# dalek-cryptography/bulletproofs

Measured on AMD Instinct MI355X. Metric: 64-bit rangeproof verifications/sec (batched), higher is better.
Workload: dtype u32 limbs (10x25.5-bit GF(2^255-19), 8x32-bit scalars mod l), u64 accumulators

## Files before the change

### bulletproofs_amd/csrc/k_rp34.hip

```cpp
#include <hip/hip_runtime.h>
#include "kernels.h"

using namespace bp;

#ifndef BP_STAGE3_WAVES
#define BP_STAGE3_WAVES 1
#endif
template <int FORM>
__global__ void __launch_bounds__(BP_BLOCK, FORM == 1 ? 1 : BP_STAGE3_WAVES) k_rp_stage3(uint32_t n_win, uint32_t nthreads_win, const vb_chunk *chunks, const ge_cached *tab,
                                                         const uint32_t *recoded, ge_ext *part, ge_cached *colc, uint32_t nthreads_exp,
                                                         rp_shape sh, fb_params prm, const uint32_t *fields, fb_digit *digits,
                                                         const uint32_t *status, uint32_t n_exp, uint32_t nthreads_rows, uint32_t lg_m, const ge_cached *tab_hi) {
    if (blockIdx.x < n_win) {
        const uint32_t tid = blockIdx.x * BP_BLOCK + threadIdx.x;
        if (tid < nthreads_win) vb_window_thread(tid, chunks, tab, recoded, part, colc, nullptr, tab_hi, sh.narrow_hi, (uint64_t)8 * sh.nproofs * sh.U);
    } else if (blockIdx.x < n_win + n_exp) {
        const uint32_t tid = (blockIdx.x - n_win) * BP_BLOCK + threadIdx.x;
        if (tid < nthreads_exp) {
            if (FORM == 1) rp_expand_b8_thread(tid, sh, prm, fields, digits, status);
            else if (FORM == 2) rp_expand_b1_thread(tid, sh, prm, fields, digits, status);
            else rp_expand_b4_thread(tid, sh, prm, fields, digits, status);
        }
    } else {
        const uint32_t tid = (blockIdx.x - n_win - n_exp) * BP_BLOCK + threadIdx.x;
        if (tid < nthreads_rows) rp_rows_thread(tid, sh, prm, lg_m, fields, digits, status);
    }
}
template __global__ void k_rp_stage3<0>(uint32_t, uint32_t, const vb_chunk *, const ge_cached *, const uint32_t *, ge_ext *, ge_cached *, uint32_t, rp_shape, fb_params,
                                        const uint32_t *, fb_digit *, const uint32_t *, uint32_t, uint32_t, uint32_t, const ge_cached *);
template __global__ void k_rp_stage3<1>(uint32_t, uint32_t, const vb_chunk *, const ge_cached *, const uint32_t *, ge_ext *, ge_cached *, uint32_t, rp_shape, fb_params,
                                        const uint32_t *, fb_digit *, const uint32_t *, uint32_t, uint32_t, uint32_t, const ge_cached *);
template __global__ void k_rp_stage3<2>(uint32_t, uint32_t, const vb_chunk *, const ge_cached *, const uint32_t *, ge_ext *, ge_cached *, uint32_t, rp_shape, fb_params,
                                        const uint32_t *, fb_digit *, const uint32_t *, uint32_t, uint32_t, uint32_t, const ge_cached *);

template <bool PAIRS>
__global__ void __attribute__((amdgpu_waves_per_eu(2, 2))) __launch_bounds__(BP_BLOCK) k_rp_exponents(uint32_t nthreads_exp, rp_shape sh, fb_params prm, const uint32_t *fields,
                                                                                                 fb_digit *digits, const uint32_t *status) {
    const uint32_t tid = blockIdx.x * BP_BLOCK + threadIdx.x;
    if (tid < nthreads_exp) {
        if (PAIRS) rp_expand_b8_thread(tid, sh, prm, fields, digits, status);
        else rp_expand_b4_thread(tid, sh, prm, fields, digits, status);
    }
}
template __global__ void k_rp_exponents<false>(uint32_t, rp_shape, fb_params, const uint32_t *, fb_digit *, const uint32_t *);
template __global__ void k_rp_exponents<true>(uint32_t, rp_shape, fb_params, const uint32_t *, fb_digit *, const uint32_t *);
__global__ void __attribute__((amdgpu_waves_per_eu(3, 3))) __launch_bounds__(BP_BLOCK) k_rp_exponents_w3(uint32_t nthreads_exp, rp_shape sh, fb_params prm, const uint32_t *fields,
                                                                                                    fb_digit *digits, const uint32_t *status) {
    const uint32_t tid = blockIdx.x * BP_BLOCK + threadIdx.x;
    if (tid < nthreads_exp) rp_expand_b8_thread(tid, sh, prm, fields, digits, status);
}

__global__ void __launch_bounds__(FB_BLOCK) k_rp_horner1(uint32_t nproofs, const ge_cached *colc, ge_ext *hq) {
    vb_horner_cached_thread(blockIdx.x * FB_BLOCK + threadIdx.x, nproofs, colc, hq);
}

template <bool R5>
__global__ void __launch_bounds__(FB_BLOCK) k_rp_horner_wide(uint32_t nproofs, const ge_cached *colc, const ge_cached *extra, uint32_t extra_stride, ge_ext *hq) {
    vb_horner_wide_thread<R5>(blockIdx.x * FB_BLOCK + threadIdx.x, nproofs, colc, extra, extra_stride, hq);
}
template __global__ void k_rp_horner_wide<false>(uint32_t, const ge_cached *, const ge_cached *, uint32_t, ge_ext *);
template __global__ void k_rp_horner_wide<true>(uint32_t, const ge_cached *, const ge_cached *, uint32_t, ge_ext *);

__device__ __forceinline__ void rp_fused_finish(uint32_t p, uint32_t nproofs, uint32_t nparts, const ge_ext *hq, const ge_ext *partial, uint32_t *fin_cnt, uint32_t *status,
                                                uint8_t *verdict, const rp_seg_tab &segs) {
    __threadfence();
    const uint32_t before = atomicAdd(fin_cnt + p, 1u);
    if (before != nparts) return;
    __threadfence();
    ge_ext acc = hq[p];
#pragma unroll 1
    for (uint32_t j = 0; j < nparts; j++) {
        const ge_ext q = partial[(uint64_t)j * nproofs + p];
        ge_add(acc, acc, q);
    }
    if (segs.n) {
        const rp_seg sg = rp_seg_lookup(segs, p);
        shared_finish_tail(p, p - sg.first, acc, status, nullptr, sg.verdict);
    } else {
        shared_finish_tail(p, acc, status, nullptr, verdict);
    }
    status[p] = 0;
    fin_cnt[p] = 0;
}
__device__ __forceinline__ void rp_walk_narrow(uint32_t L, fb_params prm, uint32_t nproofs, uint32_t nsplit, uint32_t npairs, const uint32_t *gen_ids,
                                               const fb_digit *digits, const fb_entry *table, ge_ext *partial, bool fused, const ge_ext *hq, uint32_t *fin_cnt,
                                               uint32_t *status, uint8_t *verdict, const rp_seg_tab &segs) {
    __shared__ ge_ext xch[FB_BLOCK];
    const uint32_t nsg = nsplit / FB_BLOCK, p = L / nsg, sg = L - p * nsg, lane = threadIdx.x, split = sg * FB_BLOCK + lane;
    const uint32_t per = (npairs + nsplit - 1) / nsplit;
    const uint32_t q0 = split * per, q1 = (q0 + per < npairs) ? q0 + per : npairs;
    ge_ext acc;
    fb_accum_point(acc, p, q0 < npairs ? q0 : npairs, q1, prm, nproofs, gen_ids, digits, table);
#pragma unroll 1
    for (uint32_t step = FB_BLOCK / 2; step >= 1; step >>= 1) {
        xch[lane] = acc;
        __syncthreads();
        if (lane < step) {
            const ge_ext q = xch[lane + step];
            ge_add(acc, acc, q);
        }
        __syncthreads();
    }
    if (lane == 0) {
        partial[(uint64_t)sg * nproofs + p] = acc;
        if (fused) rp_fused_finish(p, nproofs, nsg, hq, partial, fin_cnt, status, verdict, segs);
    }
}

template <int HL>
__global__ void __launch_bounds__(FB_BLOCK) k_rp_stage4(uint32_t n_hw, const uint32_t *chunk_first, const ge_ext *part, const ge_cached *colc,
                                                         ge_ext *hq, fb_params prm, uint32_t nproofs, uint32_t nblk_p, uint32_t nsplit,
                                                         uint32_t npairs, const uint32_t *gen_ids, const fb_digit *digits,
                                                         const fb_entry *table, ge_ext *partial, uint32_t walk_form, uint32_t *fin_cnt, uint32_t *status,
                                                         uint8_t *verdict, rp_seg_tab segs) {
    if (blockIdx.x < n_hw) {
            if (HL == 4) hq_horner_msm(blockIdx.x * 16 + (threadIdx.x >> 2), nproofs, colc, hq);
        else if (HL == 1) vb_horner_cached_thread(blockIdx.x * FB_BLOCK + threadIdx.x, nproofs, colc, hq);
        else {
            hw_colsum_horner_msm(blockIdx.x, chunk_first, part, hq + blockIdx.x, (walk_form & 8u) ? 4 : ((walk_form & 2u) ? 2 : 1));
            if (walk_form & 4u) {
                __threadfence();
                __syncthreads();
                if (threadIdx.x == 0) rp_fused_finish(blockIdx.x, nproofs, nsplit / FB_BLOCK, hq, partial, fin_cnt, status, verdict, segs);
            }
        }
        return;
    }
    if (HL == 64 && (walk_form & 1u)) {
        rp_walk_narrow(blockIdx.x - n_hw, prm, nproofs, nsplit, npairs, gen_ids, digits, table, partial, (walk_form & 4u) != 0, hq, fin_cnt, status, verdict, segs);
        return;
    }
    const uint32_t L = blockIdx.x - n_hw;
    uint32_t split, pblk;
    if ((nsplit & 7) == 0) {
        const uint32_t r = L & 7, rest = L >> 3;
        pblk = rest % nblk_p;
        split = r + 8 * (rest / nblk_p);
    } else {
        pblk = L % nblk_p;
        split = L / nblk_p;
    }
    const uint32_t p = pblk * FB_BLOCK + threadIdx.x;
    const uint32_t per = (npairs + nsplit - 1) / nsplit;
    const uint32_t q0 = split * per, q1 = (q0 + per < npairs) ? q0 + per : npairs;
    if (p < nproofs) fb_accum_thread(p, split, q0 < npairs ? q0 : npairs, q1, prm, nproofs, gen_ids, digits, table, partial);
}

template __global__ void k_rp_stage4<4>(uint32_t, const uint32_t *, const ge_ext *, const ge_cached *, ge_ext *, fb_params, uint32_t, uint32_t, uint32_t, uint32_t, const uint32_t *, const fb_digit *, const fb_entry *, ge_ext *, uint32_t, uint32_t *, uint32_t *, uint8_t *, rp_seg_tab);
template __global__ void k_rp_stage4<1>(uint32_t, const uint32_t *, const ge_ext *, const ge_cached *, ge_ext *, fb_params, uint32_t, uint32_t, uint32_t, uint32_t, const uint32_t *, const fb_digit *, const fb_entry *, ge_ext *, uint32_t, uint32_t *, uint32_t *, uint8_t *, rp_seg_tab);
template __global__ void k_rp_stage4<64>(uint32_t, const uint32_t *, const ge_ext *, const ge_cached *, ge_ext *, fb_params, uint32_t, uint32_t, uint32_t, uint32_t, const uint32_t *, const fb_digit *, const fb_entry *, ge_ext *, uint32_t, uint32_t *, uint32_t *, uint8_t *, rp_seg_tab);
```

### bulletproofs_amd/csrc/rangeproof.h

```cpp
#ifndef BPGPU_RANGEPROOF_H
#define BPGPU_RANGEPROOF_H
#include "keccak.h"
#include "rp_script.h"
#include "msm_fixed.h"
#include "sc25519.h"
#include "scinv.h"
#include "bucket.h"
#include "chacha20.h"

namespace bp {

#define BP_RP_MAX_K 16

#define BP_VERDICT_OK 0
#define BP_VERDICT_VERIFICATION 1
#define BP_VERDICT_FORMAT 2

struct rp_shape {
    uint32_t n, m, nm, k;
    uint32_t U;
    uint32_t proof_len;
    uint32_t nproofs;
    uint32_t shape_verdict;
    uint32_t radix5 = 0;
// ... 925 lines not shown
        else if (sh.n >= 32) { sum_2.v[0] = 0xffffffffu; sum_2.v[1] = (sh.n == 32) ? 0u : ((1u << (sh.n - 32)) - 1u); }
        else sum_2.v[0] = (1u << sh.n) - 1u;
        sc_sub(t1, z, zz);
        sc_to_mont28(dm, t1);
        sc28_montmul(dm, dm, sum_ym);
        sc_from_mont28(dl, dm);
        sc28 z3m, s2m;
        sc28_montmul(z3m, zzm, zm);
        sc_to_mont28(s2m, sum_2);
        sc28_montmul(z3m, z3m, s2m);
        sc28_montmul(z3m, z3m, sum_zm);
        sc_from_mont28(t1, z3m);
        sc_sub(dl, dl, t1);
        sc_sub(t1, dl, tx);
        sc_to_mont28(pm, t1);
        sc28_montmul(pm, cm, pm);
        sc_from_mont28(t1, pm);
        sc_add(t0, t0, t1);
        fb_recode(digits + ((uint64_t)1 * prm.nwin) * B + p, B, t0.v, prm);
    }
}

BP_HD void rp_two_pow_mont(sc28 &r, uint32_t i) {
    const sc28 T[64] = {
    {{0xcf5d3edu, 0x4305db8u, 0x676a4b2u, 0x80113d7u, 0x0622aafu, 0xfffeb21u, 0xfffffffu, 0xfffffffu, 0xfffffffu, 0x0000000u}},
    {{0xcf5d3edu, 0x73a89cbu, 0x550730cu, 0x0643d7fu, 0x0c44080u, 0xfffd642u, 0xfffffffu, 0xfffffffu, 0xfffffffu, 0x0000000u}},
    {{0xcf5d3edu, 0xd4ee1f1u, 0x3040fc0u, 0x12a90cfu, 0x1886c21u, 0xfffac84u, 0xfffffffu, 0xfffffffu, 0xfffffffu, 0x0000000u}},
    {{0xcf5d3edu, 0x977923du, 0xe6b4929u, 0x2b7376eu, 0x310c363u, 0xfff5908u, 0xfffffffu, 0xfffffffu, 0xfffffffu, 0x0000000u}},
    {{0xcf5d3edu, 0x1c8f2d5u, 0x539bbfbu, 0x5d084aeu, 0x62171e7u, 0xffeb210u, 0xfffffffu, 0xfffffffu, 0xfffffffu, 0x0000000u}},
    {{0xcf5d3edu, 0x26bb405u, 0x2d6a19eu, 0xc031f2du, 0xc42ceefu, 0xffd6420u, 0xfffffffu, 0xfffffffu, 0xfffffffu, 0x0000000u}},
    {{0xcf5d3edu, 0x3b13665u, 0xe106ce4u, 0x868542au, 0x8858900u, 0xffac841u, 0xfffffffu, 0xfffffffu, 0xfffffffu, 0x0000000u}},
    {{0xcf5d3edu, 0x63c3b25u, 0x4840370u, 0x132be26u, 0x10afd22u, 0xff59083u, 0xfffffffu, 0xfffffffu, 0xfffffffu, 0x0000000u}},
    {{0xcf5d3edu, 0xb5244a5u, 0x16b3088u, 0x2c7921du, 0x215e565u, 0xfeb2106u, 0xfffffffu, 0xfffffffu, 0xfffffffu, 0x0000000u}},
    {{0xcf5d3edu, 0x57e57a5u, 0xb398ab9u, 0x5f13a0au, 0x42bb5ebu, 0xfd6420cu, 0xfffffffu, 0xfffffffu, 0xfffffffu, 0x0000000u}},
    {{0xcf5d3edu, 0x9d67da5u, 0xed63f1au, 0xc4489e5u, 0x85756f7u, 0xfac8418u, 0xfffffffu, 0xfffffffu, 0xfffffffu, 0x0000000u}},
    {{0xcf5d3edu, 0x286c9a5u, 0x60fa7ddu, 0x8eb299cu, 0x0ae9910u, 0xf590831u, 0xfffffffu, 0xfffffffu, 0xfffffffu, 0x0000000u}},
    {{0xcf5d3edu, 0x3e761a5u, 0x4827962u, 0x2386909u, 0x15d1d42u, 0xeb21062u, 0xfffffffu, 0xfffffffu, 0xfffffffu, 0x0000000u}},
    {{0xcf5d3edu, 0x6a891a5u, 0x1681c6cu, 0x4d2e7e3u, 0x2ba25a5u, 0xd6420c4u, 0xfffffffu, 0xfffffffu, 0xfffffffu, 0x0000000u}},
    {{0xcf5d3edu, 0xc2af1a5u, 0xb336280u, 0xa07e596u, 0x574366bu, 0xac84188u, 0xfffffffu, 0xfffffffu, 0xfffffffu, 0x0000000u}},
    {{0xcf5d3edu, 0x72fb1a5u, 0xec9eea9u, 0x471e0fdu, 0xae857f8u, 0x5908310u, 0xfffffffu, 0xfffffffu, 0xfffffffu, 0x0000000u}},
    {{0xcf5d3edu, 0xd3931a5u, 0x5f706fau, 0x945d7ccu, 0x5d09b11u, 0xb210621u, 0xffffffeu, 0xfffffffu, 0xfffffffu, 0x0000000u}},
    {{0xcf5d3edu, 0x94c31a5u, 0x451379du, 0x2edc569u, 0xba12144u, 0x6420c42u, 0xffffffdu, 0xfffffffu, 0xfffffffu, 0x0000000u}},
    {{0xcf5d3edu, 0x17231a5u, 0x10598e3u, 0x63da0a3u, 0x7422da9u, 0xc841885u, 0xffffffau, 0xfffffffu, 0xfffffffu, 0x0000000u}},
    {{0xcf5d3edu, 0x1be31a5u, 0xa6e5b6eu, 0xcdd5716u, 0xe844673u, 0x908310au, 0xffffff5u, 0xfffffffu, 0xfffffffu, 0x0000000u}},
    {{0xcf5d3edu, 0x25631a5u, 0xd3fe084u, 0xa1cc3fdu, 0xd087808u, 0x2106215u, 0xfffffebu, 0xfffffffu, 0xfffffffu, 0x0000000u}},
    {{0xcf5d3edu, 0x38631a5u, 0x2e2eab0u, 0x49b9dccu, 0xa10db32u, 0x420c42bu, 0xfffffd6u, 0xfffffffu, 0xfffffffu, 0x0000000u}},
    {{0xcf5d3edu, 0x5e631a5u, 0xe28ff08u, 0x9995168u, 0x421a185u, 0x8418857u, 0xfffffacu, 0xfffffffu, 0xfffffffu, 0x0000000u}},
    {{0xcf5d3edu, 0xaa631a5u, 0x4b527b8u, 0x394b8a2u, 0x8432e2cu, 0x08310aeu, 0xfffff59u, 0xfffffffu, 0xfffffffu, 0x0000000u}},
    {{0xcf5d3edu, 0x42631a5u, 0x1cd7919u, 0x78b8715u, 0x0864779u, 0x106215du, 0xffffeb2u, 0xfffffffu, 0xfffffffu, 0x0000000u}},
    {{0xcf5d3edu, 0x72631a5u, 0xbfe1bdau, 0xf7923fau, 0x10c7a13u, 0x20c42bau, 0xffffd64u, 0xfffffffu, 0xfffffffu, 0x0000000u}},
    {{0xcf5d3edu, 0xd2631a5u, 0x05f615cu, 0xf545dc6u, 0x218df48u, 0x4188574u, 0xffffac8u, 0xfffffffu, 0xfffffffu, 0x0000000u}},
    {{0xcf5d3edu, 0x92631a5u, 0x921ec61u, 0xf0ad15cu, 0x431a9b2u, 0x8310ae8u, 0xffff590u, 0xfffffffu, 0xfffffffu, 0x0000000u}},
    {{0xcf5d3edu, 0x12631a5u, 0xaa7026bu, 0xe77b889u, 0x8633e86u, 0x06215d0u, 0xfffeb21u, 0xfffffffu, 0xfffffffu, 0x0000000u}},
    {{0xcf5d3edu, 0x12631a5u, 0xdb12e7eu, 0xd5186e3u, 0x0c6682eu, 0x0c42ba1u, 0xfffd642u, 0xfffffffu, 0xfffffffu, 0x0000000u}},
    {{0xcf5d3edu, 0x12631a5u, 0x3c586a4u, 0xb052398u, 0x18cbb7eu, 0x1885742u, 0xfffac84u, 0xfffffffu, 0xfffffffu, 0x0000000u}},
    {{0xcf5d3edu, 0x12631a5u, 0xfee36f0u, 0x66c5d00u, 0x319621eu, 0x310ae84u, 0xfff5908u, 0xfffffffu, 0xfffffffu, 0x0000000u}},
    {{0xcf5d3edu, 0x12631a5u, 0x83f9788u, 0xd3acfd2u, 0x632af5du, 0x6215d08u, 0xffeb210u, 0xfffffffu, 0xfffffffu, 0x0000000u}},
    {{0xcf5d3edu, 0x12631a5u, 0x8e258b8u, 0xad7b575u, 0xc6549dcu, 0xc42ba10u, 0xffd6420u, 0xfffffffu, 0xfffffffu, 0x0000000u}},
    {{0xcf5d3edu, 0x12631a5u, 0xa27db18u, 0x61180bbu, 0x8ca7edau, 0x8857421u, 0xffac841u, 0xfffffffu, 0xfffffffu, 0x0000000u}},
    {{0xcf5d3edu, 0x12631a5u, 0xcb2dfd8u, 0xc851747u, 0x194e8d5u, 0x10ae843u, 0xff59083u, 0xfffffffu, 0xfffffffu, 0x0000000u}},
    {{0xcf5d3edu, 0x12631a5u, 0x1c8e958u, 0x96c4460u, 0x329bcccu, 0x215d086u, 0xfeb2106u, 0xfffffffu, 0xfffffffu, 0x0000000u}},
    {{0xcf5d3edu, 0x12631a5u, 0xbf4fc58u, 0x33a9e90u, 0x65364bau, 0x42ba10cu, 0xfd6420cu, 0xfffffffu, 0xfffffffu, 0x0000000u}},
    {{0xcf5d3edu, 0x12631a5u, 0x04d2258u, 0x6d752f2u, 0xca6b495u, 0x8574218u, 0xfac8418u, 0xfffffffu, 0xfffffffu, 0x0000000u}},
    {{0xcf5d3edu, 0x12631a5u, 0x8fd6e58u, 0xe10bbb4u, 0x94d544bu, 0x0ae8431u, 0xf590831u, 0xfffffffu, 0xfffffffu, 0x0000000u}},
    {{0xcf5d3edu, 0x12631a5u, 0xa5e0658u, 0xc838d39u, 0x29a93b8u, 0x15d0863u, 0xeb21062u, 0xfffffffu, 0xfffffffu, 0x0000000u}},
    {{0xcf5d3edu, 0x12631a5u, 0xd1f3658u, 0x9693043u, 0x5351292u, 0x2ba10c6u, 0xd6420c4u, 0xfffffffu, 0xfffffffu, 0x0000000u}},
    {{0xcf5d3edu, 0x12631a5u, 0x2a19658u, 0x3347658u, 0xa6a1046u, 0x574218cu, 0xac84188u, 0xfffffffu, 0xfffffffu, 0x0000000u}},
    {{0xcf5d3edu, 0x12631a5u, 0xda65658u, 0x6cb0280u, 0x4d40badu, 0xae84319u, 0x5908310u, 0xfffffffu, 0xfffffffu, 0x0000000u}},
    {{0xcf5d3edu, 0x12631a5u, 0x3afd658u, 0xdf81ad2u, 0x9a8027bu, 0x5d08632u, 0xb210621u, 0xffffffeu, 0xfffffffu, 0x0000000u}},
    {{0xcf5d3edu, 0x12631a5u, 0xfc2d658u, 0xc524b74u, 0x34ff018u, 0xba10c65u, 0x6420c42u, 0xffffffdu, 0xfffffffu, 0x0000000u}},
    {{0xcf5d3edu, 0x12631a5u, 0x7e8d658u, 0x906acbau, 0x69fcb52u, 0x74218cau, 0xc841885u, 0xffffffau, 0xfffffffu, 0x0000000u}},
    {{0xcf5d3edu, 0x12631a5u, 0x834d658u, 0x26f6f45u, 0xd3f81c6u, 0xe843194u, 0x908310au, 0xffffff5u, 0xfffffffu, 0x0000000u}},
    {{0xcf5d3edu, 0x12631a5u, 0x8ccd658u, 0x540f45bu, 0xa7eeeadu, 0xd086329u, 0x2106215u, 0xfffffebu, 0xfffffffu, 0x0000000u}},
    {{0xcf5d3edu, 0x12631a5u, 0x9fcd658u, 0xae3fe87u, 0x4fdc87bu, 0xa10c653u, 0x420c42bu, 0xfffffd6u, 0xfffffffu, 0x0000000u}},
    {{0xcf5d3edu, 0x12631a5u, 0xc5cd658u, 0x62a12dfu, 0x9fb7c18u, 0x4218ca6u, 0x8418857u, 0xfffffacu, 0xfffffffu, 0x0000000u}},
    {{0xcf5d3edu, 0x12631a5u, 0x11cd658u, 0xcb63b90u, 0x3f6e351u, 0x843194du, 0x08310aeu, 0xfffff59u, 0xfffffffu, 0x0000000u}},
    {{0xcf5d3edu, 0x12631a5u, 0xa9cd658u, 0x9ce8cf0u, 0x7edb1c4u, 0x086329au, 0x106215du, 0xffffeb2u, 0xfffffffu, 0x0000000u}},
    {{0xcf5d3edu, 0x12631a5u, 0xd9cd658u, 0x3ff2fb1u, 0xfdb4eaau, 0x10c6534u, 0x20c42bau, 0xffffd64u, 0xfffffffu, 0x0000000u}},
    {{0xcf5d3edu, 0x12631a5u, 0x39cd658u, 0x8607534u, 0xfb68875u, 0x218ca69u, 0x4188574u, 0xffffac8u, 0xfffffffu, 0x0000000u}},
    {{0xcf5d3edu, 0x12631a5u, 0xf9cd658u, 0x1230038u, 0xf6cfc0cu, 0x43194d3u, 0x8310ae8u, 0xffff590u, 0xfffffffu, 0x0000000u}},
    {{0xcf5d3edu, 0x12631a5u, 0x79cd658u, 0x2a81642u, 0xed9e339u, 0x86329a7u, 0x06215d0u, 0xfffeb21u, 0xfffffffu, 0x0000000u}},
    {{0xcf5d3edu, 0x12631a5u, 0x79cd658u, 0x5b24255u, 0xdb3b193u, 0x0c6534fu, 0x0c42ba1u, 0xfffd642u, 0xfffffffu, 0x0000000u}},
    {{0xcf5d3edu, 0x12631a5u, 0x79cd658u, 0xbc69a7bu, 0xb674e47u, 0x18ca69fu, 0x1885742u, 0xfffac84u, 0xfffffffu, 0x0000000u}},
    {{0xcf5d3edu, 0x12631a5u, 0x79cd658u, 0x7ef4ac7u, 0x6ce87b0u, 0x3194d3fu, 0x310ae84u, 0xfff5908u, 0xfffffffu, 0x0000000u}},
    {{0xcf5d3edu, 0x12631a5u, 0x79cd658u, 0x040ab5fu, 0xd9cfa82u, 0x6329a7eu, 0x6215d08u, 0xffeb210u, 0xfffffffu, 0x0000000u}},
    {{0xcf5d3edu, 0x12631a5u, 0x79cd658u, 0x0e36c8fu, 0xb39e025u, 0xc6534fdu, 0xc42ba10u, 0xffd6420u, 0xfffffffu, 0x0000000u}},
    {{0xcf5d3edu, 0x12631a5u, 0x79cd658u, 0x228eeefu, 0x673ab6bu, 0x8ca69fbu, 0x8857421u, 0xffac841u, 0xfffffffu, 0x0000000u}},
    {{0xcf5d3edu, 0x12631a5u, 0x79cd658u, 0x4b3f3afu, 0xce741f7u, 0x194d3f6u, 0x10ae843u, 0xff59083u, 0xfffffffu, 0x0000000u}}};
    r = T[i & 63];
}
BP_HD void sc28_sub_lazy(sc28 &r, const sc28 &a, const sc28 &b) {
    const uint32_t L4[10] = {0x3d74fb4u, 0x498c697u, 0xe735960u, 0xe77a8bdu, 0x000537bu, 0u, 0u, 0u, 0u, 0x4u};
    int32_t cy = 0;
#pragma unroll
    for (int i = 0; i < 10; i++) {
        const int32_t t = (int32_t)a.v[i] - (int32_t)b.v[i] + (int32_t)L4[i] + cy;
        if (i < 9) {
            r.v[i] = (uint32_t)t & BP_M28;
            cy = t >> 28;
        } else {
            r.v[i] = (uint32_t)t;
        }
    }
}

BP_HD void rp_expand_b4_thread(uint32_t tid, rp_shape sh, fb_params prm, const uint32_t *fields, fb_digit *digits,
                               const uint32_t *status, sc *g_out = nullptr, sc *h_out = nullptr, uint32_t j_lo = 0, uint32_t j_hi = 4) {
    const uint32_t B = sh.nproofs, k = sh.k;
    const uint32_t t4 = tid / B, p = tid - t4 * B, i0 = 4 * t4;
    if (g_out) {
        for (int j = 0; j < 4; j++) {
            sc_0(g_out[j]);
            sc_0(h_out[j]);
        }
    }
    if (status[p] != 0) return;
    const fb_bias bias = fb_make_bias(prm);
    const rp_fields fl = rp_field_layout(k, sh.m);
    sc28 s_hi, sinv_hi, y_hi, t;
    {
        sc28 um, uim;
        sc28_one_mont(s_hi);
        sinv_hi = s_hi;
        y_hi = s_hi;
        for (uint32_t bb = 2; bb < k; bb++) {
            rp_load28(um, fields, B, fl.u_m + (k - 1 - bb), p);
            rp_load28(uim, fields, B, fl.uinv_m + (k - 1 - bb), p);
            const bool bit = (i0 >> bb) & 1;
            sc28 f1, f2;
#pragma unroll
            for (int q = 0; q < 10; q++) {
                f1.v[q] = bit ? um.v[q] : uim.v[q];
                f2.v[q] = bit ? uim.v[q] : um.v[q];
            }
            sc28_montmul(s_hi, s_hi, f1);
            sc28_montmul(sinv_hi, sinv_hi, f2);
            if (bit) {
                rp_load28(t, fields, B, fl.yinvp_m + bb, p);
                sc28_montmul(y_hi, y_hi, t);
            }
        }
    }
#if defined(__HIP_DEVICE_COMPILE__)
#pragma unroll 1
#endif
    for (uint32_t j = j_lo; j < j_hi; j++) {
        const uint32_t i = i0 + j;
        const uint32_t fa = (j & 1) ? fl.u_m + (k - 1) : fl.uinv_m + (k - 1), fa_c = (j & 1) ? fl.uinv_m + (k - 1) : fl.u_m + (k - 1);
        const uint32_t fb = (j & 2) ? fl.u_m + (k - 2) : fl.uinv_m + (k - 2), fb_c = (j & 2) ? fl.uinv_m + (k - 2) : fl.u_m + (k - 2);
        sc28 s, yp, r;
        sc g, h, v;
        {
            sc28 a_m;
            rp_load28(t, fields, B, fa, p);
            sc28_montmul(s, s_hi, t);
            rp_load28(t, fields, B, fb, p);
            sc28_montmul(s, s, t);
            rp_load28(a_m, fields, B, RPF_A_M, p);
            sc28_montmul(t, a_m, s);
            sc_from_mont28(v, t);
            sc minus_z;
            rp_load(minus_z, fields, B, RPF_MINUS_Z, p);
            sc_sub(g, minus_z, v);
            if (!g_out) fb_recode(digits + ((uint64_t)(2 + i) * prm.nwin) * B + p, B, g.v, prm, bias);
        }
        yp = y_hi;
        if (j & 1) {
            rp_load28(t, fields, B, fl.yinvp_m + 0, p);
            sc28_montmul(yp, yp, t);
        }
        if (j & 2) {
            rp_load28(t, fields, B, fl.yinvp_m + 1, p);
            sc28_montmul(yp, yp, t);
        }
        {
            sc28 sinv, b_m, two_m, zzzj;
            rp_load28(t, fields, B, fa_c, p);
            sc28_montmul(sinv, sinv_hi, t);
            rp_load28(t, fields, B, fb_c, p);
            sc28_montmul(sinv, sinv, t);
            const uint32_t jj = i / sh.n, ib = i - jj * sh.n;
            rp_load28(zzzj, fields, B, fl.zzzj_m + jj, p);
            rp_two_pow_mont(two_m, ib);
            sc28_montmul(r, zzzj, two_m);
            rp_load28(b_m, fields, B, RPF_B_M, p);
            sc28_montmul(t, b_m, sinv);
            sc28_sub_lazy(r, r, t);
            sc28_montmul(r, r, yp);
            sc_from_mont28(v, r);
            sc z;
            rp_load(z, fields, B, RPF_Z, p);
            sc_add(h, z, v);
        }
        if (g_out) {
            g_out[j] = g;
            h_out[j] = h;
        } else {
            fb_recode(digits + ((uint64_t)(2 + sh.nm + i) * prm.nwin) * B + p, B, h.v, prm, bias);
        }
    }
}
BP_HD void rp_expand_b1_thread(uint32_t tid, rp_shape sh, fb_params prm, const uint32_t *fields, fb_digit *digits, const uint32_t *status) {
    const uint32_t B = sh.nproofs, i = tid / B, p = tid - i * B;
    rp_expand_b4_thread((i >> 2) * B + p, sh, prm, fields, digits, status, nullptr, nullptr, i & 3, (i & 3) + 1);
}

BP_HD void rp_expand_b8_thread(uint32_t tid, rp_shape sh, fb_params prm, const uint32_t *fields, fb_digit *digits, const uint32_t *status) {
    const uint32_t B = sh.nproofs, k = sh.k;
    const uint32_t t8 = tid / B, p = tid - t8 * B, i0 = 4 * t8;
    if (status[p] != 0) return;
    const fb_bias bias = fb_make_bias(prm);
    const rp_fields fl = rp_field_layout(k, sh.m);
    sc28 s_hi, sinv_hi, y_hi, yc_hi, t;
    {
        sc28 um, uim;
        sc28_one_mont(s_hi);
        sinv_hi = s_hi;
        y_hi = s_hi;
        yc_hi = s_hi;
        for (uint32_t bb = 2; bb < k; bb++) {
            rp_load28(um, fields, B, fl.u_m + (k - 1 - bb), p);
            rp_load28(uim, fields, B, fl.uinv_m + (k - 1 - bb), p);
            const bool bit = (i0 >> bb) & 1;
            sc28 f1, f2;
#pragma unroll
            for (int q = 0; q < 10; q++) {
                f1.v[q] = bit ? um.v[q] : uim.v[q];
                f2.v[q] = bit ? uim.v[q] : um.v[q];
            }
            sc28_montmul(s_hi, s_hi, f1);
            sc28_montmul(sinv_hi, sinv_hi, f2);
            rp_load28(t, fields, B, fl.yinvp_m + bb, p);
            if (bit) sc28_montmul(y_hi, y_hi, t);
            else sc28_montmul(yc_hi, yc_hi, t);
        }
    }
#if defined(__HIP_DEVICE_COMPILE__)
#pragma unroll 1
#endif
    for (uint32_t j = 0; j < 4; j++) {
        const uint32_t i = i0 + j, im = sh.nm - 1 - i;
        const uint32_t fa = (j & 1) ? fl.u_m + (k - 1) : fl.uinv_m + (k - 1), fa_c = (j & 1) ? fl.uinv_m + (k - 1) : fl.u_m + (k - 1);
        const uint32_t fb = (j & 2) ? fl.u_m + (k - 2) : fl.uinv_m + (k - 2), fb_c = (j & 2) ? fl.uinv_m + (k - 2) : fl.u_m + (k - 2);
        sc28 s, sinv;
        rp_load28(t, fields, B, fa, p);
        sc28_montmul(s, s_hi, t);
        rp_load28(t, fields, B, fb, p);
        sc28_montmul(s, s, t);
        rp_load28(t, fields, B, fa_c, p);
        sc28_montmul(sinv, sinv_hi, t);
        rp_load28(t, fields, B, fb_c, p);
        sc28_montmul(sinv, sinv, t);
#if defined(__HIP_DEVICE_COMPILE__)
#pragma unroll 1
#endif
        for (uint32_t side = 0; side < 2; side++) {
            const uint32_t idx = side ? im : i, lo = side ? (3u - j) : j;
            sc28 sg, sh_, yp, r;
#pragma unroll
            for (int q = 0; q < 10; q++) {
                sg.v[q] = side ? sinv.v[q] : s.v[q];
                sh_.v[q] = side ? s.v[q] : sinv.v[q];
                yp.v[q] = side ? yc_hi.v[q] : y_hi.v[q];
            }
            sc g, h, v;
            {
                sc28 a_m;
                rp_load28(a_m, fields, B, RPF_A_M, p);
                sc28_montmul(t, a_m, sg);
                sc_from_mont28(v, t);
                sc minus_z;
                rp_load(minus_z, fields, B, RPF_MINUS_Z, p);
                sc_sub(g, minus_z, v);
                fb_recode(digits + ((uint64_t)(2 + idx) * prm.nwin) * B + p, B, g.v, prm, bias);
            }
            if (lo & 1) {
                rp_load28(t, fields, B, fl.yinvp_m + 0, p);
                sc28_montmul(yp, yp, t);
            }
            if (lo & 2) {
                rp_load28(t, fields, B, fl.yinvp_m + 1, p);
                sc28_montmul(yp, yp, t);
            }
            {
                sc28 b_m, two_m, zzzj;
                const uint32_t jj = idx / sh.n, ib = idx - jj * sh.n;
                rp_load28(zzzj, fields, B, fl.zzzj_m + jj, p);
                rp_two_pow_mont(two_m, ib);
                sc28_montmul(r, zzzj, two_m);
                rp_load28(b_m, fields, B, RPF_B_M, p);
                sc28_montmul(t, b_m, sh_);
                sc28_sub_lazy(r, r, t);
                sc28_montmul(r, r, yp);
                sc_from_mont28(v, r);
                sc z;
                rp_load(z, fields, B, RPF_Z, p);
                sc_add(h, z, v);
                fb_recode(digits + ((uint64_t)(2 + sh.nm + idx) * prm.nwin) * B + p, B, h.v, prm, bias);
            }
        }
    }
}

}
#endif
```

Measured before the change: 6.006 million.

## Add restructured b8 exponent expansion with shared prefix products and lazy reduction

Replaces the b8 exponent-expansion thread with a new variant. It builds the high-bit s, s^-1 and y-power prefixes once per group of four indices, derives the 2^i·z terms by shifting instead of multiplying, and fuses the final addition with canonical reduction. Digit recoding now uses funnel shifts over a 9-word biased value. The KEEP template variant precomputes the lower-level products to save multiplies at the cost of more registers, while the w3 variant reloads them instead to keep register pressure down.

```diff
diff --git a/bulletproofs_amd/csrc/k_rp34.hip b/bulletproofs_amd/csrc/k_rp34.hip
--- a/bulletproofs_amd/csrc/k_rp34.hip
+++ b/bulletproofs_amd/csrc/k_rp34.hip
@@ -38,7 +38,7 @@
                                                                                                  fb_digit *digits, const uint32_t *status) {
     const uint32_t tid = blockIdx.x * BP_BLOCK + threadIdx.x;
     if (tid < nthreads_exp) {
-        if (PAIRS) rp_expand_b8_thread(tid, sh, prm, fields, digits, status);
+        if (PAIRS) rp_expand_b8w_thread<true>(tid, sh, prm, fields, digits, status);
         else rp_expand_b4_thread(tid, sh, prm, fields, digits, status);
     }
 }
@@ -47,7 +47,7 @@
 __global__ void __attribute__((amdgpu_waves_per_eu(3, 3))) __launch_bounds__(BP_BLOCK) k_rp_exponents_w3(uint32_t nthreads_exp, rp_shape sh, fb_params prm, const uint32_t *fields,
                                                                                                     fb_digit *digits, const uint32_t *status) {
     const uint32_t tid = blockIdx.x * BP_BLOCK + threadIdx.x;
-    if (tid < nthreads_exp) rp_expand_b8_thread(tid, sh, prm, fields, digits, status);
+    if (tid < nthreads_exp) rp_expand_b8w_thread<false>(tid, sh, prm, fields, digits, status);
 }
 
 __global__ void __launch_bounds__(FB_BLOCK) k_rp_horner1(uint32_t nproofs, const ge_cached *colc, ge_ext *hq) {
diff --git a/bulletproofs_amd/csrc/rangeproof.h b/bulletproofs_amd/csrc/rangeproof.h
--- a/bulletproofs_amd/csrc/rangeproof.h
+++ b/bulletproofs_amd/csrc/rangeproof.h
@@ -1251,5 +1251,228 @@
     }
 }
 
-}
+BP_HD void sc28_carry(sc28 &r, const sc28 &x) {
+    uint32_t c = 0;
+#pragma unroll
+    for (int i = 0; i < 9; i++) {
+        const uint32_t s = x.v[i] + c;
+        r.v[i] = s & BP_M28;
+        c = s >> 28;
+    }
+    r.v[9] = x.v[9] + c;
+}
+BP_HD void sc28_shl(sc28 &r, const sc28 &x, uint32_t e) {
+    r.v[0] = (x.v[0] << e) & BP_M28;
+#pragma unroll
+    for (int i = 1; i < 9; i++) r.v[i] = ((x.v[i] << e) & BP_M28) | (x.v[i - 1] >> (28 - e));
+    r.v[9] = (x.v[9] << e) | (x.v[8] >> (28 - e));
+}
+BP_HD void sc28_select(sc28 &r, bool c, const sc28 &a, const sc28 &b) {
+#pragma unroll
+    for (int i = 0; i < 10; i++) r.v[i] = c ? a.v[i] : b.v[i];
+}
+BP_HD void sc_add_lazy_canonical(sc &r, const sc28 &x, const sc28 &c) {
+    const uint32_t C[5] = {BP_SC28_C0, BP_SC28_C1, BP_SC28_C2, BP_SC28_C3, BP_SC28_C4};
+    uint32_t t[10], cy = 0;
+#pragma unroll
+    for (int i = 0; i < 9; i++) {
+        const uint32_t s = x.v[i] + c.v[i] + cy;
+        t[i] = s & BP_M28;
+        cy = s >> 28;
+    }
+    const uint32_t q = x.v[9] + c.v[9] + cy;
+    int32_t b = 0;
+#pragma unroll
+    for (int i = 0; i < 9; i++) {
+        const int32_t d = (int32_t)t[i] - (i < 5 ? (int32_t)(q * C[i]) : 0) + b;
+        t[i] = (uint32_t)d & BP_M28;
+        b = d >> 28;
+    }
+    const bool neg = b < 0;
+    uint32_t k = 0;
+#pragma unroll
+    for (int i = 0; i < 9; i++) {
+        const uint32_t s = t[i] + ((i < 5 && neg) ? C[i] : 0u) + k;
+        t[i] = s & BP_M28;
+        k = s >> 28;
+    }
+    t[9] = k;
+    r.v[0] = t[0] | (t[1] << 28);
+    r.v[1] = (t[1] >> 4) | (t[2] << 24);
+    r.v[2] = (t[2] >> 8) | (t[3] << 20);
+    r.v[3] = (t[3] >> 12) | (t[4] << 16);
+    r.v[4] = (t[4] >> 16) | (t[5] << 12);
+    r.v[5] = (t[5] >> 20) | (t[6] << 8);
+    r.v[6] = (t[6] >> 24) | (t[7] << 4);
+    r.v[7] = t[8] | (t[9] << 28);
+}
+BP_HD uint32_t rp_funnel_shr(uint32_t hi, uint32_t lo, uint32_t sh ) {
+#if defined(__HIP_DEVICE_COMPILE__)
+    return __builtin_amdgcn_alignbit(hi, lo, sh);
+#else
+    return (uint32_t)((((uint64_t)hi << 32) | lo) >> sh);
 #endif
+}
+BP_HD void rp_recode9(fb_digit *digits , uint64_t stride, const uint32_t s[8], fb_params prm, const fb_bias &bias) {
+    uint32_t r[9], carry = 0;
+#pragma unroll
+    for (int i = 0; i < 9; i++) {
+        const uint64_t t = (uint64_t)(i < 8 ? s[i] : 0u) + bias.k[i] + carry;
+        r[i] = (uint32_t)t;
+        carry = (uint32_t)(t >> 32);
+    }
+    const uint32_t W = prm.W, mask = (1u << W) - 1u;
+    for (uint32_t win = 0; win < prm.nwin; win++) {
+        digits[(uint64_t)win * stride] = (fb_digit)(r[0] & mask);
+#pragma unroll
+        for (int i = 0; i < 8; i++) r[i] = rp_funnel_shr(r[i + 1], r[i], W);
+        r[8] >>= W;
+    }
+}
+template <bool KEEP>
+BP_HD void rp_expand_b8w_thread(uint32_t tid, rp_shape sh, fb_params prm, const uint32_t *fields, fb_digit *digits, const uint32_t *status) {
+    const uint32_t B = sh.nproofs, k = sh.k;
+    const uint32_t t8 = tid / B, p = tid - t8 * B, i0 = 4 * t8, i1 = sh.nm - 4 - i0;
+    if (status[p] != 0) return;
+    const fb_bias bias = fb_make_bias(prm);
+    const rp_fields fl = rp_field_layout(k, sh.m);
+    sc28 s_hi, sinv_hi, y_hi, yc_hi;
+    {
+        sc28 um, uim, yq;
+        sc28_one_mont(s_hi);
+        sinv_hi = s_hi;
+#pragma unroll
+        for (int q = 0; q < 10; q++) y_hi.v[q] = (q == 0);
+        yc_hi = y_hi;
+        rp_load28(um, fields, B, fl.u_m + (k - 3), p);
+        rp_load28(uim, fields, B, fl.uinv_m + (k - 3), p);
+        rp_load28(yq, fields, B, fl.yinvp_m + 2, p);
+        for (uint32_t bb = 2; bb < k; bb++) {
+            const uint32_t nb = bb + 1 < k ? bb + 1 : bb;
+            sc28 um_n, uim_n, yq_n;
+            rp_load28(um_n, fields, B, fl.u_m + (k - 1 - nb), p);
+            rp_load28(uim_n, fields, B, fl.uinv_m + (k - 1 - nb), p);
+            rp_load28(yq_n, fields, B, fl.yinvp_m + nb, p);
+            const bool bit = (i0 >> bb) & 1;
+            sc28 f1, f2;
+            sc28_select(f1, bit, um, uim);
+            sc28_select(f2, bit, uim, um);
+            sc28_montmul(s_hi, s_hi, f1);
+            sc28_montmul(sinv_hi, sinv_hi, f2);
+            if (bit) sc28_montmul(y_hi, y_hi, yq);
+            else sc28_montmul(yc_hi, yc_hi, yq);
+            um = um_n;
+            uim = uim_n;
+            yq = yq_n;
+        }
+    }
+    sc28 zz0, zz1;
+    {
+        sc28 zzzj, two_m;
+        const uint32_t jj0 = i0 / sh.n, jj1 = i1 / sh.n;
+        rp_load28(zzzj, fields, B, fl.zzzj_m + jj0, p);
+        rp_two_pow_mont(two_m, i0 - jj0 * sh.n);
+        sc28_montmul(zz0, zzzj, two_m);
+        sc28_carry(zz0, zz0);
+        rp_load28(zzzj, fields, B, fl.zzzj_m + jj1, p);
+        rp_two_pow_mont(two_m, i1 - jj1 * sh.n);
+        sc28_montmul(zz1, zzzj, two_m);
+        sc28_carry(zz1, zz1);
+    }
+    sc28 sA, sB, iA, iB, y0B, y1A, u0, ui0, yi0;
+    if (KEEP) {
+        sc28 u1, ui1, yi1;
+        rp_load28(u1, fields, B, fl.u_m + (k - 2), p);
+        rp_load28(ui1, fields, B, fl.uinv_m + (k - 2), p);
+        rp_load28(yi1, fields, B, fl.yinvp_m + 1, p);
+        rp_load28(u0, fields, B, fl.u_m + (k - 1), p);
+        rp_load28(ui0, fields, B, fl.uinv_m + (k - 1), p);
+        rp_load28(yi0, fields, B, fl.yinvp_m + 0, p);
+        sc28_montmul(sA, s_hi, ui1);
+        sc28_montmul(sB, s_hi, u1);
+        sc28_montmul(iA, sinv_hi, u1);
+        sc28_montmul(iB, sinv_hi, ui1);
+        sc28_montmul(y0B, y_hi, yi1);
+        sc28_montmul(y1A, yc_hi, yi1);
+    }
+#if defined(__HIP_DEVICE_COMPILE__)
+#pragma unroll 1
+#endif
+    for (uint32_t j = 0; j < 4; j++) {
+        const bool b0 = j & 1, b1 = j & 2;
+        const uint32_t idx0 = i0 + j, idx1 = i1 + 3u - j;
+        sc28 s, sinv;
+        {
+            sc a, mz;
+            sc28 na, mz28, s1, inv1, f0, f0c, t0, t1;
+            rp_load(a, fields, B, RPF_A, p);
+            rp_load(mz, fields, B, RPF_MINUS_Z, p);
+            if (KEEP) {
+                sc28_select(s1, b1, sB, sA);
+                sc28_select(inv1, b1, iB, iA);
+                sc28_select(f0, b0, u0, ui0);
+                sc28_select(f0c, b0, ui0, u0);
+            } else {
+                sc28 f1, f1c;
+                rp_load28(f1, fields, B, (b1 ? fl.u_m : fl.uinv_m) + (k - 2), p);
+                rp_load28(f1c, fields, B, (b1 ? fl.uinv_m : fl.u_m) + (k - 2), p);
+                rp_load28(f0, fields, B, (b0 ? fl.u_m : fl.uinv_m) + (k - 1), p);
+                rp_load28(f0c, fields, B, (b0 ? fl.uinv_m : fl.u_m) + (k - 1), p);
+                sc28_montmul(s1, s_hi, f1);
+                sc28_montmul(inv1, sinv_hi, f1c);
+            }
+            sc28_montmul(s, s1, f0);
+            sc28_montmul(sinv, inv1, f0c);
+            sc_neg(a, a);
+            sc28_from_sc(na, a);
+            sc28_from_sc(mz28, mz);
+            sc28_montmul(t0, na, s);
+            sc28_montmul(t1, na, sinv);
+            sc g0, g1;
+            sc_add_lazy_canonical(g0, t0, mz28);
+            sc_add_lazy_canonical(g1, t1, mz28);
+            rp_recode9(digits + ((uint64_t)(2 + idx0) * prm.nwin) * B + p, B, g0.v, prm, bias);
+            rp_recode9(digits + ((uint64_t)(2 + idx1) * prm.nwin) * B + p, B, g1.v, prm, bias);
+        }
+        {
+            sc z;
+            sc28 b_m, z28, ya, yb, ys, yt, yp0, yp1, zs0, zs1, t0, t1;
+            rp_load28(b_m, fields, B, RPF_B_M, p);
+            rp_load(z, fields, B, RPF_Z, p);
+            if (KEEP) {
+                sc28_select(ya, b1, y0B, y_hi);
+                sc28_select(yb, b1, yc_hi, y1A);
+                yt = yi0;
+            } else {
+                sc28 yi1;
+                rp_load28(yi1, fields, B, fl.yinvp_m + 1, p);
+                rp_load28(yt, fields, B, fl.yinvp_m + 0, p);
+                sc28_select(ys, b1, y_hi, yc_hi);
+                sc28_montmul(yi1, ys, yi1);
+                sc28_select(ya, b1, yi1, y_hi);
+                sc28_select(yb, b1, yc_hi, yi1);
+            }
+            sc28_select(ys, b0, ya, yb);
+            sc28_montmul(yt, ys, yt);
+            sc28_select(yp0, b0, yt, ya);
+            sc28_select(yp1, b0, yb, yt);
+            sc28_montmul(t0, b_m, sinv);
+            sc28_montmul(t1, b_m, s);
+            sc28_shl(zs0, zz0, j);
+            sc28_shl(zs1, zz1, 3u - j);
+            sc28_sub_lazy(t0, zs0, t0);
+            sc28_sub_lazy(t1, zs1, t1);
+            sc28_montmul(t0, t0, yp0);
+            sc28_montmul(t1, t1, yp1);
+            sc28_from_sc(z28, z);
+            sc h0, h1;
+            sc_add_lazy_canonical(h0, t0, z28);
+            sc_add_lazy_canonical(h1, t1, z28);
+            rp_recode9(digits + ((uint64_t)(2 + sh.nm + idx0) * prm.nwin) * B + p, B, h0.v, prm, bias);
+            rp_recode9(digits + ((uint64_t)(2 + sh.nm + idx1) * prm.nwin) * B + p, B, h1.v, prm, bias);
+        }
+    }
+}
+
+}
+#endif
```

After: 6.065 million, median of 6. No clear change (+1.0%).
